# ChrisHird/ZLIB

Measured on AMD Instinct MI355X. Metric: GiB/s raw input compressed (deflate level 6), higher is better.
Workload: dtype u8

## Files before the change

zlib_amd/csrc/zgpu_lz_sorted.hip:

```cpp
#include "zgpu_common.h"
#include "zgpu_engine.h"
#define ZGPU_PARSE_HEADER_ONLY
#include "zgpu_lz_parse.h"
#include <cstdlib>
#include "../../include/zamd_gpu.h"

#include <atomic>
static std::atomic<int> g_inject_sort_fault{0};
extern "C" __attribute__((visibility("default"))) void zgpu_debug_inject_sort_fault(void) { g_inject_sort_fault.store(1); }

namespace zgpu {

__device__ inline uint32_t lds_off(const void *p) { return (uint32_t)(uintptr_t)(const __attribute__((address_space(3))) void *)p; }
__device__ inline void lds_st32(uint32_t a, uint32_t v) { asm volatile("ds_write_b32 %0, %1" ::"v"(a), "v"(v) : "memory"); }
__device__ inline void lds_st16(uint32_t a, uint32_t v) { asm volatile("ds_write_b16 %0, %1" ::"v"(a), "v"(v) : "memory"); }
__device__ inline void lds_max32(uint32_t a, uint32_t v) { asm volatile("ds_max_u32 %0, %1" ::"v"(a), "v"(v) : "memory"); }
__device__ inline uint32_t lds_ld32(uint32_t a) { uint32_t v; asm volatile("ds_read_b32 %0, %1\n\ts_waitcnt lgkmcnt(0)" : "=v"(v) : "v"(a) : "memory"); return v; }
__device__ inline uint32_t lds_ld16(uint32_t a) { uint32_t v; asm volatile("ds_read_u16 %0, %1\n\ts_waitcnt lgkmcnt(0)" : "=v"(v) : "v"(a) : "memory"); return v; }

__device__ inline void lds_st8(uint32_t a, uint32_t v) { asm volatile("ds_write_b8 %0, %1" ::"v"(a), "v"(v) : "memory"); }
__device__ inline uint32_t lds_ld8(uint32_t a) { uint32_t v; asm volatile("ds_read_u8 %0, %1\n\ts_waitcnt lgkmcnt(0)" : "=v"(v) : "v"(a) : "memory"); return v; }

constexpr uint32_t kSuperS = 1024;

// ... 514 lines not shown
    uint64_t lo; uint32_t n;
    chunk_span(g, c, lo, n);
    const uint8_t *src = g.in + lo;
    const uint16_t *S = S_all + (size_t)c * kSStride + kSPad;
    const unsigned long long *hd = reinterpret_cast<const unsigned long long *>(heads_all + (size_t)c * kHeadStride);
    uint2 *rec = recs + (size_t)c * kChunkMax;
    const uint32_t npos = n >= 3 ? n - 2 : 0;
    const uint32_t base = chunk_base(g, c);
    stage_chunk<kM2Threads>(src, n, d32, tid);
    if (tid == 0) *work_next = 0;
    for (uint32_t q2 = npos + tid; q2 < n; q2 += kM2Threads) rec[q2] = make_uint2((uint32_t)src[q2] << 24, 0);
    __syncthreads();

    const uint32_t chainF = cfg.chain, chainQ = cfg.chain >> 2, dbase = lds_off(d32), nblk = (npos + 63) >> 6;
    const uint16_t *hb = reinterpret_cast<const uint16_t *>(heads_all + (size_t)c * kHeadStride + kHeadWords);
    auto grab = [&]() { uint32_t b = 0; if (lane == 0) b = atomicAdd(work_next, 1u); return (uint32_t)__builtin_amdgcn_readfirstlane(b); };
    uint32_t blk = grab(), p_nx = 0, below_nx = 0;
    unsigned long long m_nx = 0;
    if (blk < nblk) { const uint32_t wi = (blk << 6) + lane; p_nx = wi < npos ? S[wi] : 0; m_nx = hd[blk]; below_nx = hb[blk]; }
    while (blk < nblk) {
        const uint32_t wi = (blk << 6) + lane;
        const bool valid = wi < npos;
        const uint32_t p = p_nx, below = below_nx;
        const unsigned long long m = m_nx;
        const uint32_t blk_nx = grab();
        if (blk_nx < nblk) { const uint32_t wn = (blk_nx << 6) + lane; p_nx = wn < npos ? S[wn] : 0; m_nx = hd[blk_nx]; below_nx = hb[blk_nx]; }
        uint32_t avail = 0;
        {
            const unsigned long long mine = m & ((2ull << lane) - 1);
            const uint32_t rank = mine ? (uint32_t)__builtin_clzll(mine) - (63 - lane) : lane + below;
            if (valid) avail = rank < chainF ? rank : chainF;
        }
        const int w = (int)(p + base);
        int thr = (w - (int)kMaxDist > 1 ? w - (int)kMaxDist : 1) - (int)base;
        const int thr_next = (w - (int)kMaxDist + 1 > 1 ? w - (int)kMaxDist + 1 : 1) - (int)base;
        if (cfg.strategy == kRle && thr < (int)p - 1) thr = (int)p - 1;
        uint32_t best = kMinMatch - 1, key_seen = 0, snapkey = 0;
        uint32_t scan2 = (uint32_t)d8[p + 1] | ((uint32_t)d8[p + 2] << 8);
        uint32_t boff = dbase + best - 1;
        unsigned long long amask = mask_gt_u32(avail, 0u);
        bool snap_taken = false;
        const uint16_t *sp = S + wi;
        lds_st32(slot + lane * 4, 0);
        lds_st16(pw + lane * 2, p);
        uint32_t tail = 0;
        const uint32_t lanebits = lane << 16, dummy = ring + (kRing - 1) * 4;
        M3_STAT(5, __popcll(__builtin_amdgcn_ballot_w64(valid)));

        auto fold = [&](uint32_t kcur) {
            const uint32_t cnt = tail < 64 ? tail : 64;
            M3_STAT(3, 1);
            tail = (uint32_t)__builtin_amdgcn_readfirstlane(tail - cnt);
            if (lane < cnt) {
                const uint32_t e = lds_ld32(ring + ((tail + lane) << 2));
                const uint32_t q = e & 0xffffu, o = (e >> 16) & 63u;
                const uint32_t k = kcur - ((kcur - (e >> 22)) & 1023u);
                const uint32_t po = lds_ld16(pw + o * 2), look = n - po, cap = look < kMaxMatch ? look : kMaxMatch, nice = cfg.nice < look ? cfg.nice : look;
                uint32_t l = 0, x;
                for (;;) {
                    x = lds_ld32u(dbase + q + l) ^ lds_ld32u(dbase + po + l);
                    M3_STAT(4, 1);
                    if (x != 0 || l + 4 >= cap) break;
                    l += 4;
                }
                uint32_t len = x ? l + ((uint32_t)__builtin_ctz(x) >> 3) : l + 4;
                len = len < cap ? len : cap;
                if (len >= kMinMatch) {
                    const uint32_t key = len >= nice ? (0x80000000u | ((4095u - k) << 16) | len) : ((len << 16) | (4095u - k));
                    lds_max32(slot + o * 4, key);
                }
            }
            const uint32_t key = lds_ld32(slot + lane * 4);
            if (key != key_seen) {
                key_seen = key;
                best = (key >> 31) ? key & 0x1ffu : key >> 16;
                boff = dbase + best - 1;
                scan2 = (uint32_t)d8[p + best - 1] | ((uint32_t)d8[p + best] << 8);
            }
            amask &= ~mask_lt_i32((int)key, 0);
        };

        auto group = [&](uint32_t k0) -> uint64_t {
            int gi = (int)wi - 4 - (int)k0, gsel;
            gi = gi < -(int)kSPad ? -(int)kSPad : gi;
            asm("v_cndmask_b32_e64 %0, %1, %2, %3" : "=v"(gsel) : "v"(-(int)kSPad), "v"(gi), "s"(amask));
            return reinterpret_cast<const U64u *>(S + gsel)->v;
        };
        uint64_t cq = group(0);
        uint32_t k = 0;
        const uint32_t snapK = chainQ & ~3u, snapJ = chainQ & 3u;
        for (;; k += 4) {
            if (amask == 0) break;
            if (k == chainQ) {
                while (tail) fold(k);
                snapkey = key_seen; snap_taken = true;
            } else if ((k & (ZGPU_M3_PERIOD - 1)) == 0) { while (tail) fold(k); }
            const uint64_t cqn = group(k + 4);
#pragma unroll
            for (uint32_t j = 0; j < 4; j++) {
                const uint32_t q = (uint32_t)(cq >> (48 - 16 * j)) & 0xffffu;
                if (j != 0 && j == snapJ && k == snapK) {
                    while (tail) fold(k + j);
                    snapkey = key_seen; snap_taken = true;
                }
                uint32_t b0, b1;
                lds_ld2bytes(boff + q, b0, b1);
                amask &= mask_le_i32(thr, (int)q);
                if (k == 0 && j == 0) thr = thr_next;
                const unsigned long long m = amask & mask_eq_u32(b0 | (b1 << 8), scan2);
                M3_STAT(0, 1); M3_STAT(1, __popcll(amask)); M3_STAT(2, __popcll(m));
                if (m) {
                    stack_push(m, (uint32_t)__builtin_amdgcn_readfirstlane(ring + (tail << 2)), dummy, q | lanebits | ((k + j) << 22));
                    tail = (uint32_t)__builtin_amdgcn_readfirstlane(tail + (uint32_t)__popcll(m));
                    if (tail >= 64) fold(k + j);
                }
                amask &= mask_gt_u32(avail, k + j + 1);
            }
            cq = cqn;
        }
        while (tail) fold(k);
        if (!snap_taken) snapkey = key_seen;
        if (valid) {
            uint32_t full = 0, snap = 0, flags = 0;
            if (key_seen) {
                const uint32_t kb = 4095u - ((key_seen >> 31) ? (key_seen >> 16) & 0xfffu : key_seen & 0xfffu);
                full = best | ((p - (uint32_t)sp[-1 - (int)kb]) << 9);
            }
            if (snapkey) {
                const uint32_t ks = 4095u - ((snapkey >> 31) ? (snapkey >> 16) & 0xfffu : snapkey & 0xfffu);
                const uint32_t sl = (snapkey >> 31) ? snapkey & 0x1ffu : snapkey >> 16;
                snap = sl | ((p - (uint32_t)sp[-1 - (int)ks]) << 9);
            }
            if (p + base == kWSize + kMaxDist && avail != 0 && (uint32_t)sp[-1] + base == kWSize) flags = 1;
            rec[p] = make_uint2(full | ((uint32_t)d8[p] << 24), snap | (flags << 24));
        }
        blk = blk_nx;
    }
}

#ifndef ZGPU_WTRIG
#define ZGPU_WTRIG 48
#endif
#ifndef ZGPU_WBLK
#define ZGPU_WBLK 64
#endif
#ifndef ZGPU_WNEU_SHIFT
#define ZGPU_WNEU_SHIFT 0
#endif
#ifndef ZGPU_WFOLD_AT
#define ZGPU_WFOLD_AT 64
#endif
constexpr uint32_t kWFoldAt = ZGPU_WFOLD_AT;
constexpr uint32_t kWThreads = 512, kWWaves = kWThreads / 64, kWBlk = ZGPU_WBLK, kWTrig = ZGPU_WTRIG, kWNeuShift = ZGPU_WNEU_SHIFT;
constexpr uint32_t kWNeuBytes = (kChunkMax >> kWNeuShift) / 8;
constexpr uint32_t kWOffLcnt = kM3DataLds + 16 + kWNeuBytes + kWWaves * kM3WaveLds;
constexpr uint32_t kWLds = kWOffLcnt + kP2Wins * 4;
static_assert(2 * kWLds <= 160 * 1024, "two walker workgroups per CU");
enum : uint32_t { W_NEED = 0, W_LIMBO = 1, W_READY = 2, W_SEARCH = 3, W_DONE = 4 };
#ifdef ZGPU_WALK_STATS
__device__ unsigned long long walk_stats[8];
extern "C" __attribute__((visibility("default"))) void zgpu_debug_walk_stats(unsigned long long *out, int reset)
{
    unsigned long long z[8] = {};
    hipMemcpyFromSymbol(out, HIP_SYMBOL(walk_stats), sizeof z);
    if (reset) hipMemcpyToSymbol(HIP_SYMBOL(walk_stats), z, sizeof z);
}
#define W_STAT(i, v) do { const unsigned long long v_ = (unsigned long long)(v); if (lane == 0) atomicAdd(&walk_stats[i], v_); } while (0)
__device__ unsigned long long walk_log_stats[2];
extern "C" __attribute__((visibility("default"))) void zgpu_debug_walk_log_stats(unsigned long long *out, int reset)
{
    unsigned long long z[2] = {};
    hipMemcpyFromSymbol(out, HIP_SYMBOL(walk_log_stats), sizeof z);
    if (reset) hipMemcpyToSymbol(HIP_SYMBOL(walk_log_stats), z, sizeof z);
}
#else
#define W_STAT(i, v) do { } while (0)
#endif
#ifdef ZGPU_WALK_TIME
__device__ unsigned long long walk_time[8];
extern "C" __attribute__((visibility("default"))) void zgpu_debug_walk_time(unsigned long long *out, int reset)
{
    unsigned long long z[8] = {};
    hipMemcpyFromSymbol(out, HIP_SYMBOL(walk_time), sizeof z);
    if (reset) hipMemcpyToSymbol(HIP_SYMBOL(walk_time), z, sizeof z);
}
#define W_T0() unsigned long long wt_prev = __builtin_readcyclecounter(), wt_fold = 0, wt_lds = 0, wt_take = 0, wt_acc[8] = {0, 0, 0, 0, 0, 0, 0, 0}
#define W_T(i) do { const unsigned long long t_ = __builtin_readcyclecounter(); wt_acc[i] += t_ - wt_prev - ((i) == 1 ? wt_fold + wt_lds + wt_take : 0); \
                    if ((i) == 1) { wt_acc[2] += wt_fold; wt_acc[3] += wt_lds; wt_acc[7] += wt_take; } wt_fold = wt_lds = wt_take = 0; wt_prev = t_; } while (0)
#define W_TF(stmt) do { const unsigned long long f0_ = __builtin_readcyclecounter(); stmt; wt_fold += __builtin_readcyclecounter() - f0_; } while (0)
#define W_TL(stmt) do { const unsigned long long f0_ = __builtin_readcyclecounter(); stmt; wt_lds += __builtin_readcyclecounter() - f0_; } while (0)
#define W_TK(stmt) do { const unsigned long long f0_ = __builtin_readcyclecounter(); asm volatile("s_waitcnt vmcnt(0)" ::: "memory"); stmt; wt_take += __builtin_readcyclecounter() - f0_; } while (0)
#define W_TEND() do { if (lane == 0) for (int i_ = 0; i_ < 8; i_++) atomicAdd(&walk_time[i_], wt_acc[i_]); } while (0)
#else
#define W_T0() do { } while (0)
#define W_T(i) do { } while (0)
#define W_TF(stmt) stmt
#define W_TL(stmt) stmt
#define W_TK(stmt) stmt
#define W_TEND() do { } while (0)
#endif
__device__ inline uint32_t add_w1(uint32_t b, uint32_t w) { uint32_t r; asm("v_add_u32_sdwa %0, %1, %2 dst_sel:DWORD dst_unused:UNUSED_PAD src0_sel:DWORD src1_sel:WORD_1" : "=v"(r) : "v"(b), "v"(w)); return r; }
__device__ inline uint32_t add_w0(uint32_t b, uint32_t w) { uint32_t r; asm("v_add_u32_sdwa %0, %1, %2 dst_sel:DWORD dst_unused:UNUSED_PAD src0_sel:DWORD src1_sel:WORD_0" : "=v"(r) : "v"(b), "v"(w)); return r; }
__device__ inline uint32_t or_w1(uint32_t b, uint32_t w) { uint32_t r; asm("v_or_b32_sdwa %0, %1, %2 dst_sel:DWORD dst_unused:UNUSED_PAD src0_sel:DWORD src1_sel:WORD_1" : "=v"(r) : "v"(b), "v"(w)); return r; }
__device__ inline uint32_t and_or(uint32_t w, uint32_t m, uint32_t b) { uint32_t r; asm("v_and_or_b32 %0, %1, %2, %3" : "=v"(r) : "v"(w), "s"(m), "v"(b)); return r; }
__device__ inline uint32_t sel_mask(unsigned long long m, uint32_t if_set, uint32_t if_clear) { uint32_t r; asm("v_cndmask_b32_e64 %0, %1, %2, %3" : "=v"(r) : "v"(if_clear), "v"(if_set), "s"(m)); return r; }

template <uint32_t T>
__device__ inline void tile_exits(uint8_t *pl, const uint32_t *gm, const uint32_t *gs, uint32_t h0, uint32_t h1, uint32_t nent, uint16_t *exits, uint32_t tid)
{
    constexpr uint32_t kWords = kChunkMax / 32;
    static_assert(kWords % T == 0 && T % 64 == 0 && T <= 1024, "workgroup size");
    uint32_t *HAS = reinterpret_cast<uint32_t *>(pl);
    uint16_t *wcnt = reinterpret_cast<uint16_t *>(pl + kWords * 4);
    uint32_t *wtot = reinterpret_cast<uint32_t *>(pl + kWords * 6);
    uint16_t *N = reinterpret_cast<uint16_t *>(pl + kWords * 6 + 64);
    constexpr uint32_t kCapNodes = (kM3DataLds - (kWords * 6 + 64)) / 2;
    static_assert(kCapNodes < 0x8000u && kCapNodes > kTileH1 / 3, "a path's game starts are three positions apart at least; different paths' need not be");
    const uint32_t lane = tid & 63, wave = tid >> 6;
    constexpr uint32_t per = kWords / T;
    uint32_t sum = 0, cnt[per];
#pragma unroll
    for (uint32_t i = 0; i < per; i++) {
        const uint32_t w = tid * per + i, v = __hip_atomic_load(gs + w, __ATOMIC_RELAXED, __HIP_MEMORY_SCOPE_AGENT);
        HAS[w] = v; cnt[i] = (uint32_t)__builtin_popcount(v); sum += cnt[i];
    }
    uint32_t x = sum;
#pragma unroll
    for (int d = 1; d < 64; d <<= 1) { const uint32_t y = __shfl_up(x, d); if ((int)lane >= d) x += y; }
    if (lane == 63) wtot[wave] = x;
    __syncthreads();
    uint32_t b = x - sum;
    for (uint32_t w = 0; w < wave; w++) b += wtot[w];
#pragma unroll
    for (uint32_t i = 0; i < per; i++) { wcnt[tid * per + i] = (uint16_t)b; b += cnt[i]; }
    __syncthreads();
    uint32_t nn = 0;
    for (uint32_t w = 0; w < T / 64; w++) nn += wtot[w];
    auto rank_of = [&](uint32_t p) { return (uint32_t)wcnt[p >> 5] + (uint32_t)__builtin_popcount(HAS[p >> 5] & ~(~0u << (p & 31u))); };
    if (nn > kCapNodes) {
        for (uint32_t k = tid; k < kTileExitStride; k += T) {
            uint32_t v = 0;
            if (k < nent) {
                const uint32_t e = h0 + k;
                uint32_t p = e < h1 ? next_bit(HAS, e, kWords) : kNone, x = e > h1 ? e : h1;
                while (p != kNone && p < h1) {
                    const uint32_t gv = __hip_atomic_load(gm + p, __ATOMIC_RELAXED, __HIP_MEMORY_SCOPE_AGENT), q = p + (gv >> 24) + ((gv >> 15) & 511u);
                    x = q > h1 ? q : h1;
                    p = q < h1 ? next_bit(HAS, q, kWords) : kNone;
                }
                v = x - h1;
            }
            exits[k] = (uint16_t)v;
        }
        return;
    }
    constexpr uint32_t kExit = 0x8000u;
    for (uint32_t p0 = h0 & ~31u; p0 < h1; p0 += T * 8) {
        uint32_t gv[8];
#pragma unroll
        for (uint32_t u = 0; u < 8; u++) { const uint32_t p = p0 + u * T + tid; gv[u] = p < h1 ? __hip_atomic_load(gm + p, __ATOMIC_RELAXED, __HIP_MEMORY_SCOPE_AGENT) : 0u; }
#pragma unroll
        for (uint32_t u = 0; u < 8; u++) {
            const uint32_t p = p0 + u * T + tid;
            if (p < h1 && ((HAS[p >> 5] >> (p & 31u)) & 1u)) {
                const uint32_t q = p + (gv[u] >> 24) + ((gv[u] >> 15) & 511u);
                uint32_t v = kExit | (q > h1 ? q - h1 : 0u);
                if (q < h1) { const uint32_t t = next_bit(HAS, q, kWords); if (t != kNone && t < h1) v = rank_of(t); }
                N[rank_of(p)] = (uint16_t)v;
            }
        }
    }
    __syncthreads();
    for (;;) {
        bool more = false;
        for (uint32_t i = tid; i < nn; i += T) {
            const uint32_t v = N[i];
            if (!(v & kExit)) { const uint32_t w = N[v]; N[i] = (uint16_t)w; more = more || !(w & kExit); }
        }
        if (!__syncthreads_or(more)) break;
    }
    for (uint32_t k = tid; k < kTileExitStride; k += T) {
        uint32_t v = 0;
        if (k < nent) {
            const uint32_t e = h0 + k, t = e < h1 ? next_bit(HAS, e, kWords) : kNone;
            v = (t == kNone || t >= h1) ? (e > h1 ? e - h1 : 0u) : ((uint32_t)N[rank_of(t)] & 0x7fffu);
        }
        exits[k] = (uint16_t)v;
    }
}

static_assert(kP2LogLdsBytes <= kWOffLcnt, "the parse works in the memory of the chunk bytes, the neutral bitmap and the rings");
template <int MODE>
__global__ void __launch_bounds__(kWThreads, kWThreads / 128) walk_kernel(ChunkGeom g, LevelCfg cfg, const uint16_t *__restrict__ S_all, const uint32_t *__restrict__ ir_all,
                                                            uint32_t *__restrict__ gm_all, uint32_t *__restrict__ gs_all, uint32_t *__restrict__ tokens, ChunkMeta *meta, TileGeom tg)
{
    static_assert(MODE == 1 || MODE == 2, "a chunk or a tile");
    constexpr bool FUSE = MODE == 1, TILE = MODE == 2;
    static_assert(!FUSE || kWNeuShift == 0, "a log holds kP2Win games: a position must start one game at most, so every neutral position is claimed");
    extern __shared__ __attribute__((aligned(16))) uint32_t lds[];
    uint32_t *d32 = lds;
    uint32_t *ctrl = lds + kM3DataLds / 4;
    uint32_t *NEU = ctrl + 4;
    uint32_t *lcnt = lds + kWOffLcnt / 4;
    const uint8_t *d8 = reinterpret_cast<const uint8_t *>(d32);
    const uint32_t c = blockIdx.x, tid = threadIdx.x, lane = tid & 63, wave = tid >> 6;
    const uint32_t ring = (uint32_t)__builtin_amdgcn_readfirstlane(lds_off(lds) + kM3DataLds + 16 + kWNeuBytes + wave * kM3WaveLds), slot = ring + kRing * 4, pw = slot + 64 * 4;
    uint64_t lo; uint32_t n;
    chunk_span(g, c, lo, n);
    const uint8_t *src = g.in + lo;
    const uint16_t *S = S_all + (size_t)c * kSStride + kSPad;
    const uint32_t *ir = ir_all + (size_t)c * kChunkMax;
    uint32_t *gm = gm_all + (size_t)c * kChunkMax, *gs = gs_all + (size_t)c * (kChunkMax / 32);
    uint32_t *lrec = gm; uint16_t *lpos = reinterpret_cast<uint16_t *>(gs_all) + (size_t)c * kChunkMax;
    uint32_t th0 = 0, th1 = n, tnent = 0, tnent_all = 0, nil_local = ~0u;
    uint32_t base = chunk_base(g, c);
    if (TILE) {
        uint64_t wb; uint32_t nl;
        tile_span(g, tg, c, wb, nl, th0, th1, tnent);
        tnent_all = tnent;
        if (tnent > th1 - th0) tnent = th1 - th0;
        base = (tg.abs0_nil && tg.abs0 + wb == 0) ? 0u : 1u;
        if (tg.nil_pos >= wb && tg.nil_pos - wb < kChunkMax) nil_local = (uint32_t)(tg.nil_pos - wb);
    }
    const uint32_t npos = n >= 3 ? n - 2 : 0;
    stage_chunk<kWThreads>(src, n, d32, tid);
    for (uint32_t i = tid; i < kChunkMax / 32; i += kWThreads) { if (i < kWNeuBytes / 4) NEU[i] = 0; if (!FUSE) gs[i] = 0; }
    if (tid < 8) d32[(kChunkMax + 64) / 4 + tid] = 0xffffffffu;
    if (tid == 0) ctrl[0] = 0;
    if (FUSE && tid < kP2Wins) lcnt[tid] = 0;
    __syncthreads();
    int slide_at;
    {
        const int room = (int)(2 * kWSize - base), b0 = (int)n < room ? (int)n : room;
        const int a = b0 - (int)kMinLookahead + 1, b = (int)(kWSize + kMaxDist) - (int)base;
        slide_at = a > b ? a : b;
    }
    const uint32_t chainF = cfg.chain, chainQ = cfg.chain >> 2, dbase = lds_off(d32), nblk = TILE ? tnent + (th1 - th0 - tnent + kWBlk - 1) / kWBlk : (n + kWBlk - 1) / kWBlk;
    const uint32_t wlim = TILE ? th1 : n;
    const bool vexact = (chainF & 7u) != 0 || (chainQ & 7u) != 0 || cfg.strategy == kRle;
    uint32_t lanebits = lane << 16;
    const uint32_t dummy = ring + (kRing - 1) * 4;
    uint32_t st = W_NEED, x = 0, handL = kMinMatch - 1, handM = 0, handD = 0, gstart = 0;
    uint32_t irx = 0, irn = 0, irE = 0, irl = 0;
    bool haveE = false;
    uint32_t rem = 0, best = kMinMatch - 1, key_seen = 0, sentinel = 0, scan2 = 0, boff = dbase + 1;
    int gi = -(int)kSPad;
    uint32_t firstb = 0;
    uint4 G0 = make_uint4(0, 0, 0, 0), G1 = G0, G2 = G0, G3 = G0, F0 = G0, F1 = G0, F2 = G0, F3 = G0;
    uint32_t left = 0;
    bool cont = false;
    unsigned long long amask = 0, jmask = 0;
    uint32_t tail = 0;

    auto fold = [&]() {
        const uint32_t cnt = tail < 64 ? tail : 64;
        W_STAT(5, 1); W_STAT(6, cnt);
        tail = (uint32_t)__builtin_amdgcn_readfirstlane(tail - cnt);
        if (lane < cnt) {
            const uint32_t e = lds_ld32(ring + ((tail + lane) << 2));
            const uint32_t q = e & 0xffffu, o = (e >> 16) & 63u;
            const uint32_t po = lds_ld16(pw + o * 2), look = n - po, cap = look < kMaxMatch ? look : kMaxMatch, nice = cfg.nice < look ? cfg.nice : look;
            const bool reach = po - q <= kMaxDist - ((e >> 22) & 1u ? 0u : 1u) && q + base >= 1u;
            uint32_t l = 0, xa, xb;
            for (;;) {
                lds_cmp8(dbase + q + l, dbase + po + l, xa, xb);
                if ((xa | xb) != 0 || l + 8 >= cap) break;
                l += 8;
            }
            uint32_t len = xa ? l + ((uint32_t)__builtin_ctz(xa) >> 3) : xb ? l + 4 + ((uint32_t)__builtin_ctz(xb) >> 3) : l + 8;
            len = len < cap ? len : cap;
            if (len >= kMinMatch && reach) lds_max32(slot + o * 4, (len >= nice && len > (e >> 23)) ? (0x80000000u | (q << 9) | len) : ((len << 16) | q));
        }
        const uint32_t key = lds_ld32(slot + lane * 4);
        if (key != key_seen) {
            key_seen = key;
            best = (key >> 31) ? key & 0x1ffu : key >> 16;
            boff = dbase + best - 1;
            scan2 = (uint32_t)d8[x + best - 1] | ((uint32_t)d8[x + best] << 16);
        }
        amask &= ~mask_lt_i32((int)key, 0);
    };
    auto gload = [&](int gi) -> uint4 { gi = gi < -(int)kSPad ? -(int)kSPad : gi; return reinterpret_cast<const U128u *>(S + gi)->v; };

    W_T0();
    W_T(3);
    for (;;) {
        while (tail) fold();
        W_T(4);
        if (cont && (key_seen >> 31)) cont = false;
        const bool fin = st == W_SEARCH && !(((amask | jmask) >> lane) & 1ull) && !cont;
        W_STAT(2, 1); W_STAT(3, __popcll(__builtin_amdgcn_ballot_w64(fin || st == W_LIMBO || st == W_NEED)));
        if (st == W_LIMBO) { irx = irl; st = W_READY; }
        uint32_t y = 0, irY = 0;
        bool toN = false, haveIr = false;
        if (fin) {
            uint32_t len = kMinMatch - 1, dist = 0;
            if (key_seen != sentinel) {
                const bool nz = key_seen >> 31;
                len = nz ? key_seen & 0x1ffu : key_seen >> 16;
                dist = x - (nz ? (key_seen >> 9) & 0xffffu : key_seen & 0xffffu);
            }
            if (len <= 5 && (cfg.strategy == kFiltered || (len == kMinMatch && dist > kTooFar))) len = kMinMatch - 1;
            bool emit = false;
            if (len > handL) {
                if (handL < kMinMatch) gstart = x;
                handL = len; handD = dist; handM = x;
                if (len < cfg.lazy && x + 1 < npos) { x = x + 1; irx = irn; st = W_READY; }
                else emit = true;
                haveE = false;
            } else if (handL >= kMinMatch) emit = true;
            else { y = x + 1; irY = irn; toN = haveIr = true; }
            if (emit) {
                const uint32_t rec = ((handM - gstart) << 24) | (handL << 15) | handD;
                if (FUSE) {
                    const uint32_t w = gstart / kP2Win, at = w * kP2Win + atomicAdd(&lcnt[w], 1u);
                    lrec[at] = rec; lpos[at] = (uint16_t)gstart;
                } else {
                    gm[gstart] = rec;
                    atomicOr(&gs[gstart >> 5], 1u << (gstart & 31u));
                }
                y = handM + handL; irY = irE; haveIr = haveE; toN = true;
                handL = kMinMatch - 1;
            }
        }
        if (toN) {
            st = W_NEED;
            if (y < wlim) {
                const uint32_t yc = y >> kWNeuShift, bit = 1u << (yc & 31u);
                const bool meet = (y & ((1u << kWNeuShift) - 1u)) == 0;
                if (!meet || !(atomicOr(&NEU[yc >> 5], bit) & bit)) {
                    x = y;
                    if (haveIr) { irx = irY; st = W_READY; }
                    else { irl = y < npos ? ir[y] : 0; st = W_LIMBO; W_STAT(7, 1); }
                }
            }
        }
        W_T(5);
        {
            const unsigned long long nm = __builtin_amdgcn_ballot_w64(st == W_NEED);
            if (nm) {
                const int first = __builtin_ctzll(nm);
                uint32_t b0 = 0;
                if ((int)lane == first) b0 = atomicAdd(&ctrl[0], (uint32_t)__popcll(nm));
                b0 = (uint32_t)__builtin_amdgcn_readlane((int)b0, first);
                if (st == W_NEED) {
                    const uint32_t b = b0 + __builtin_amdgcn_mbcnt_hi((uint32_t)(nm >> 32), __builtin_amdgcn_mbcnt_lo((uint32_t)nm, 0));
                    if (b >= nblk) st = W_DONE;
                    else {
                        const uint32_t y2 = TILE ? (b < tnent ? th0 + b : th0 + tnent + (b - tnent) * kWBlk) : b * kWBlk, bit = 1u << ((y2 >> kWNeuShift) & 31u);
                        if (!(atomicOr(&NEU[(y2 >> kWNeuShift) >> 5], bit) & bit)) { x = y2; handL = kMinMatch - 1; irl = y2 < npos ? ir[y2] : 0; st = W_LIMBO; }
                    }
                }
            }
        }
        W_T(6);
        bool fresh = false;
        if (st == W_READY) {
            const uint32_t seed = handL, idx = irx & 0xffffu, rank = irx >> 16, budget = seed >= cfg.good ? (chainQ ? chainQ : 0xffffu) : chainF;
            uint32_t avail = (x < npos && seed < cfg.lazy) ? (rank < budget ? rank : budget) : 0;
            irn = x + 1 < npos ? ir[x + 1] : 0;
            if (seed >= kMinMatch) { const uint32_t E = handM + handL; irE = E < npos ? ir[E] : 0; haveE = true; }
            if (TILE) {
                if (x == nil_local && avail != 0 && x - (uint32_t)S[idx - 1] == kMaxDist) avail = 0;
                if (cfg.strategy == kHuffmanOnly) avail = 0;
                if (cfg.strategy == kRle && avail != 0) avail = x - (uint32_t)S[idx - 1] == 1 ? 1u : 0u;
            }
            else if (x + base == kWSize + kMaxDist && avail != 0 && (int)x >= slide_at && (uint32_t)S[idx - 1] + base == kWSize) avail = 0;
            best = seed; sentinel = (seed << 16) | 0xffffu; key_seen = sentinel; boff = dbase + best - 1;
            scan2 = (uint32_t)d8[x + best - 1] | ((uint32_t)d8[x + best] << 16);
            lds_st32(slot + lane * 4, sentinel);
            lds_st16(pw + lane * 2, x);
            lanebits = (lane << 16) | (seed << 23);
            rem = avail; firstb = 1u << 22;
            gi = (int)idx - 8;
            st = W_SEARCH;
            fresh = avail != 0;
            W_STAT(4, 1);
        }
        if (cont) { cont = false; fresh = true; }
        jmask = __builtin_amdgcn_ballot_w64(fresh);
        if (fresh) {
            F0 = gload(gi);
            if (rem > 8) F1 = gload(gi - 8);
            if (rem > 16) F2 = gload(gi - 16);
            if (rem > 24) F3 = gload(gi - 24);
            gi -= 32;
        }
        W_T(0);
        if (__builtin_amdgcn_ballot_w64(st != W_DONE) == 0) { W_TEND(); break; }
        const unsigned long long smask = __builtin_amdgcn_ballot_w64(st == W_SEARCH);
        const uint32_t idle = (uint32_t)__popcll(__builtin_amdgcn_ballot_w64(st == W_LIMBO || st == W_NEED));

        for (bool first = true;; first = false) {
            const unsigned long long amask0 = amask;
            if (amask) {
                W_STAT(0, 1);
                const uint32_t scan0 = sel_mask(amask0, scan2, 0xffffffffu);
                uint32_t bb[8], a[8], boff_e;
                boff_e = boff;
                if (!vexact) {
                    const uint32_t boff_i = dbase + kChunkMax + 8u;
                    G0.x = sel_mask(amask0, G0.x, 0u); G0.y = sel_mask(amask0, G0.y, 0u); G0.z = sel_mask(amask0, G0.z, 0u); G0.w = sel_mask(amask0, G0.w, 0u);
                    boff_e = sel_mask(amask0, boff, boff_i);
                }
                a[0] = add_w1(boff_e, G0.w); a[1] = add_w0(boff_e, G0.w); a[2] = add_w1(boff_e, G0.z); a[3] = add_w0(boff_e, G0.z);
                a[4] = add_w1(boff_e, G0.y); a[5] = add_w0(boff_e, G0.y); a[6] = add_w1(boff_e, G0.x); a[7] = add_w0(boff_e, G0.x);
                if (vexact) {
                    const uint32_t nv = rem < 8 ? rem : 8, sent = dbase + (scan2 ? kChunkMax + 8u : kChunkMax + 64u + 8u);
#pragma unroll
                    for (uint32_t j = 0; j < 8; j++) a[j] = j < nv ? a[j] : sent;
                }
                uint32_t hi[8];
                W_TL(
                    asm volatile("ds_read_u8 %0, %16\n\tds_read_u8 %8, %16 offset:1\n\tds_read_u8 %1, %17\n\tds_read_u8 %9, %17 offset:1\n\t"
                                 "ds_read_u8 %2, %18\n\tds_read_u8 %10, %18 offset:1\n\tds_read_u8 %3, %19\n\tds_read_u8 %11, %19 offset:1\n\t"
                                 "ds_read_u8 %4, %20\n\tds_read_u8 %12, %20 offset:1\n\tds_read_u8 %5, %21\n\tds_read_u8 %13, %21 offset:1\n\t"
                                 "ds_read_u8 %6, %22\n\tds_read_u8 %14, %22 offset:1\n\tds_read_u8 %7, %23\n\tds_read_u8 %15, %23 offset:1\n\t"
                                 "s_waitcnt lgkmcnt(0)"
                                 : "=&v"(bb[0]), "=&v"(bb[1]), "=&v"(bb[2]), "=&v"(bb[3]), "=&v"(bb[4]), "=&v"(bb[5]), "=&v"(bb[6]), "=&v"(bb[7]),
                                   "=&v"(hi[0]), "=&v"(hi[1]), "=&v"(hi[2]), "=&v"(hi[3]), "=&v"(hi[4]), "=&v"(hi[5]), "=&v"(hi[6]), "=&v"(hi[7])
                                 : "v"(a[0]), "v"(a[1]), "v"(a[2]), "v"(a[3]), "v"(a[4]), "v"(a[5]), "v"(a[6]), "v"(a[7]) : "memory"));
#pragma unroll
                for (uint32_t j = 0; j < 8; j++) bb[j] |= hi[j] << 16;
                W_STAT(1, __popcll(amask0) * 8);
                const uint32_t lf = lanebits | firstb;
                unsigned long long mm[8];
                uint32_t total = 0;
#pragma unroll
                for (uint32_t j = 0; j < 8; j++) { mm[j] = mask_eq_u32(bb[j], scan0); total += (uint32_t)__popcll(mm[j]); }
                auto entry_of = [&](uint32_t j) -> uint32_t {
                    const uint32_t wd = j < 2 ? G0.w : j < 4 ? G0.z : j < 6 ? G0.y : G0.x, lb = j == 0 ? lf : lanebits;
                    return (j & 1) ? and_or(wd, 0xffffu, lb) : or_w1(lb, wd);
                };
                if (total) {
                    if (tail + total > kRing - 1) { while (tail) W_TF(fold()); }
                    if (total <= kRing - 1) {
                        uint32_t ta[8], te[8];
#pragma unroll
                        for (uint32_t j = 0; j < 8; j++) {
                            ta[j] = stack_slot(mm[j], ring + (tail << 2)); te[j] = entry_of(j);
                            tail += (uint32_t)__popcll(mm[j]);
                        }
                        tail = (uint32_t)__builtin_amdgcn_readfirstlane(tail);
                        unsigned long long sv;
                        asm volatile("s_mov_b64 %0, exec\n\t"
                                     "s_mov_b64 exec, %17\n\tds_write_b32 %1, %9\n\ts_mov_b64 exec, %18\n\tds_write_b32 %2, %10\n\t"
                                     "s_mov_b64 exec, %19\n\tds_write_b32 %3, %11\n\ts_mov_b64 exec, %20\n\tds_write_b32 %4, %12\n\t"
                                     "s_mov_b64 exec, %21\n\tds_write_b32 %5, %13\n\ts_mov_b64 exec, %22\n\tds_write_b32 %6, %14\n\t"
                                     "s_mov_b64 exec, %23\n\tds_write_b32 %7, %15\n\ts_mov_b64 exec, %24\n\tds_write_b32 %8, %16\n\t"
                                     "s_mov_b64 exec, %0"
                                     : "=&s"(sv)
                                     : "v"(ta[0]), "v"(ta[1]), "v"(ta[2]), "v"(ta[3]), "v"(ta[4]), "v"(ta[5]), "v"(ta[6]), "v"(ta[7]),
                                       "v"(te[0]), "v"(te[1]), "v"(te[2]), "v"(te[3]), "v"(te[4]), "v"(te[5]), "v"(te[6]), "v"(te[7]),
                                       "s"(mm[0]), "s"(mm[1]), "s"(mm[2]), "s"(mm[3]), "s"(mm[4]), "s"(mm[5]), "s"(mm[6]), "s"(mm[7]) : "memory");
                    } else {
#pragma unroll
                        for (uint32_t j = 0; j < 8; j++) {
                            if (mm[j]) {
                                stack_push(mm[j], (uint32_t)__builtin_amdgcn_readfirstlane(ring + (tail << 2)), dummy, entry_of(j));
                                tail = (uint32_t)__builtin_amdgcn_readfirstlane(tail + (uint32_t)__popcll(mm[j]));
                                if (tail >= kWFoldAt) W_TF(fold());
                            }
                        }
                    }
                    while (tail >= kWFoldAt) W_TF(fold());
                }
                amask &= mask_gt_u32(rem, 8u);
                firstb = sel_mask(amask0, 0u, firstb);
            }
            G0 = G1; G1 = G2; G2 = G3;
            left = left ? left - 1 : 0;
            if (first && jmask) {
                W_TK(if ((jmask >> lane) & 1ull) { G0 = F0; G1 = F1; G2 = F2; G3 = F3; left = 4; });
            }
            rem = sel_mask(amask0, rem > 8 ? rem - 8 : 0, rem);
            {
                const unsigned long long cm = amask & mask_eq_u32(left, 0u);
                cont = cont || ((cm >> lane) & 1ull);
                amask &= ~cm;
            }
            amask |= jmask; jmask = 0;
            if (amask == 0 || (uint32_t)__popcll(smask & ~amask) + idle >= kWTrig) break;
        }
        W_T(1);
    }
    if (TILE) {
        __syncthreads();
        tile_exits<kWThreads>(reinterpret_cast<uint8_t *>(lds), gm, gs, th0, th1, tnent_all, tg.exits + (size_t)c * kTileExitStride, tid);
    }
    if (FUSE) {
        __syncthreads();
#ifdef ZGPU_WALK_STATS
        if (tid < kP2Wins) { atomicAdd(&walk_log_stats[0], (unsigned long long)lcnt[tid]); atomicMax(&walk_log_stats[1], (unsigned long long)lcnt[tid]); }
#endif
        constexpr uint32_t kP2Threads = kWThreads;
        constexpr bool LITE = true, FUSED = true, TILE = false, LOG = true;
        const uint2 *recs = nullptr;
        const uint32_t *gmv_all = nullptr, *gsv_all = nullptr;
        uint8_t *pl = reinterpret_cast<uint8_t *>(lds);
        uint16_t *const J = reinterpret_cast<uint16_t *>(pl + kP2OffJ);
        uint32_t *const HAS = reinterpret_cast<uint32_t *>(pl + kP2OffHAS), *const MARK = reinterpret_cast<uint32_t *>(pl + kP2OffMARK), *const COV = reinterpret_cast<uint32_t *>(pl + kP2OffCOV),
                 *const MAT = reinterpret_cast<uint32_t *>(pl + kP2OffMAT), *const wbase = reinterpret_cast<uint32_t *>(pl + kP2OffWbase), *const VIS = reinterpret_cast<uint32_t *>(pl + kP2OffVIS),
                 *const EXITS = reinterpret_cast<uint32_t *>(pl + kP2OffEXITS), *const wave_tot = reinterpret_cast<uint32_t *>(pl + kP2OffWtot);
        uint32_t &sh_entry = *reinterpret_cast<uint32_t *>(pl + kP2OffEntry), &sh_exit = *reinterpret_cast<uint32_t *>(pl + kP2OffEntry + 4);
        uint16_t *const END = reinterpret_cast<uint16_t *>(pl + kP2OffEND);
#include "zgpu_lz_parse_body.inc"
    }
}

struct __attribute__((packed, aligned(1))) U128b { uint4 v; };
enum : uint32_t { F_IR = 0, F_GROUP, F_CAND, F_EXT, F_DONE };

__device__ inline uint32_t first_diff16(uint4 a, uint4 b)
{
    const uint64_t x0 = (((uint64_t)(a.y ^ b.y)) << 32) | (a.x ^ b.x), x1 = (((uint64_t)(a.w ^ b.w)) << 32) | (a.z ^ b.z);
    return x0 ? (uint32_t)__builtin_ctzll(x0) >> 3 : x1 ? 8 + ((uint32_t)__builtin_ctzll(x1) >> 3) : 16u;
}

__device__ __noinline__ uint4 tail16(const uint8_t *in, uint32_t o, uint64_t safe_end)
{
    uint32_t v[4] = {0, 0, 0, 0};
    for (uint32_t k = 0; k < 16 && (uint64_t)o + k < safe_end; k++) v[k >> 2] |= (uint32_t)in[o + k] << (8 * (k & 3));
    return make_uint4(v[0], v[1], v[2], v[3]);
}

__global__ void __launch_bounds__(64) fast_kernel(ChunkGeom g, LevelCfg cfg, const uint16_t *__restrict__ S_all, const uint32_t *__restrict__ ir_all, uint8_t *G_all,
                                                   uint32_t *__restrict__ tokens, ChunkMeta *meta, uint32_t lanes)
{
    const uint32_t c = blockIdx.x * lanes + threadIdx.x;
    const bool live = threadIdx.x < lanes && c < g.nchunks;
    const uint32_t cc = live ? c : 0;
    uint64_t lo; uint32_t n;
    chunk_span(g, cc, lo, n);
    const uint8_t *in = g.in + lo;
    const uint64_t safe_end = g.in_bytes - lo;
    const uint16_t *S = S_all + (size_t)cc * kSStride + kSPad;
    const uint32_t *ir = ir_all + (size_t)cc * kChunkMax;
    uint8_t *G = G_all + (size_t)cc * kGStride + kGPad;
    uint32_t *tok = tokens + (size_t)cc * kChunkMax;
    const uint8_t *dummy = reinterpret_cast<const uint8_t *>(S_all);
    const uint32_t base = chunk_base(g, cc);
    uint32_t off = 0, ntok = 0, blk_tok0 = 0, nblk = 0, nostore = 0, block_start = 0;
    auto cut_block = [&](uint32_t p_end) {
        if (off != 0 && block_start + base < kWSize) nostore |= 1u << nblk;
        nblk++; blk_tok0 = ntok; block_start = p_end;
    };
    const uint32_t room = 2 * kWSize - base;
    uint32_t buffered = n < room ? n : room;
    uint32_t p = 0, st = live ? F_IR : F_DONE;
    auto token_top = [&]() {
        if (buffered - p < kMinLookahead) {
            if ((int)(p + base) - (int)off >= (int)(kWSize + kMaxDist)) off += kWSize;
            buffered = n;
            if (n == p) { cut_block(p); st = F_DONE; }
        }
    };
    if (live) token_top();
    uint32_t irw[8] = {0, 0, 0, 0, 0, 0, 0, 0};
    uint4 scan = make_uint4(0, 0, 0, 0), cb[4] = {scan, scan, scan, scan};
    bool fresh = false;
    uint32_t idx = 0, rank = 0, j0 = 0, chain = 0, best = 0, mstart = 0, cap = 0, nice = 0, look = 0, ncand = 0, cand[4] = {0, 0, 0, 0}, extl = 0;
    int w = 0, limit = 0;
    bool first = true, over = false, lastg = false;

    auto setup_search = [&](uint32_t iv) {
        idx = iv & 0xffffu; rank = iv >> 16;
        w = (int)(p + base) - (int)off; limit = w > (int)kMaxDist ? w - (int)kMaxDist : 0;
        cap = look < kMaxMatch ? look : kMaxMatch; nice = cfg.nice < look ? cfg.nice : look;
        chain = cfg.chain; best = kMinMatch - 1; first = true; over = false; lastg = false; j0 = 0; ncand = 0;
    };

    for (;;) {
        if (__builtin_amdgcn_ballot_w64(st != F_DONE) == 0) break;
        constexpr uint32_t kNone = 0xffffffffu;
        const uint8_t *a0 = dummy, *a1 = dummy, *a2 = dummy, *a3 = dummy;
        uint32_t o0 = kNone, o1 = kNone, o2 = kNone, o3 = kNone, o4 = kNone;
        const bool want_ir = st == F_IR || (st == F_GROUP && fresh);
        if (want_ir) { a2 = reinterpret_cast<const uint8_t *>(ir + p); a3 = reinterpret_cast<const uint8_t *>(ir + p + 4); o4 = p; }
        if (st == F_GROUP) { const int at = (int)idx - (int)j0 - 8; a0 = reinterpret_cast<const uint8_t *>(S + at); a1 = G + at; }
        if (st == F_CAND) { o0 = cand[0]; o1 = ncand > 1 ? cand[1] : kNone; o2 = ncand > 2 ? cand[2] : kNone; o3 = ncand > 3 ? cand[3] : kNone; }
        if (st == F_EXT) { o0 = cand[0] + extl; o1 = p + extl; }
        const bool u0 = o0 != kNone && (uint64_t)o0 + 16 > safe_end, u1 = o1 != kNone && (uint64_t)o1 + 16 > safe_end, u2 = o2 != kNone && (uint64_t)o2 + 16 > safe_end,
                   u3 = o3 != kNone && (uint64_t)o3 + 16 > safe_end, u4 = o4 != kNone && (uint64_t)o4 + 16 > safe_end;
        if (o0 != kNone && !u0) a0 = in + o0;
        if (o1 != kNone && !u1) a1 = in + o1;
        if (o2 != kNone && !u2) a2 = in + o2;
        if (o3 != kNone && !u3) a3 = in + o3;
        const uint8_t *a4 = (o4 != kNone && !u4) ? in + o4 : dummy;
        uint4 r0 = reinterpret_cast<const U128b *>(a0)->v, r1 = reinterpret_cast<const U128b *>(a1)->v, r2 = reinterpret_cast<const U128b *>(a2)->v,
              r3 = reinterpret_cast<const U128b *>(a3)->v, r4 = reinterpret_cast<const U128b *>(a4)->v;
        if (__builtin_amdgcn_ballot_w64(u0 || u1 || u2 || u3 || u4)) {
            if (u0) r0 = tail16(in, o0, safe_end);
            if (u1) r1 = tail16(in, o1, safe_end);
            if (u2) r2 = tail16(in, o2, safe_end);
            if (u3) r3 = tail16(in, o3, safe_end);
            if (u4) r4 = tail16(in, o4, safe_end);
        }

        bool eval = false, fin = false;
        if (want_ir) {
            irw[0] = r2.x; irw[1] = r2.y; irw[2] = r2.z; irw[3] = r2.w; irw[4] = r3.x; irw[5] = r3.y; irw[6] = r3.z; irw[7] = r3.w;
            scan = r4;
        }
        if (st == F_IR) {
            look = n - p;
            if (look < kMinMatch) { first = true; fin = true; }
            else { setup_search(irw[0]); if (rank == 0) fin = true; else st = F_GROUP; }
        } else if (st == F_GROUP) {
            fresh = false;
            const uint64_t fl = ((uint64_t)r1.y << 32) | r1.x;
            uint32_t used = 0;
            const uint32_t room4 = chain < 4 ? chain : 4;
            for (uint32_t t = 0; t < 8; t++) {
                if (ncand >= room4) break;
                if (j0 + t + 1 > rank) { lastg = true; break; }
                used = t + 1;
                const uint32_t slot = 7 - t;
                if (!((fl >> (8 * slot)) & 1u)) continue;
                const uint32_t wd = slot >= 6 ? r0.w : slot >= 4 ? r0.z : slot >= 2 ? r0.y : r0.x, q = (slot & 1) ? wd >> 16 : wd & 0xffffu;
                const int wq = (int)(q + base) - (int)off;
                bool stop = wq <= 0;
                if (first) { stop = stop || (uint32_t)(w - wq) > kMaxDist; first = first && stop; }
                else stop = stop || wq <= limit;
                if (stop) { lastg = true; break; }
                cand[3] = ncand == 3 ? q : cand[3]; cand[2] = ncand == 2 ? q : cand[2]; cand[1] = ncand == 1 ? q : cand[1]; cand[0] = ncand == 0 ? q : cand[0];
                ncand++;
            }
            j0 += used;
            if (ncand) st = F_CAND;
            else if (lastg || j0 >= rank) fin = true;
        } else if (st == F_CAND) {
            cb[0] = r0; cb[1] = r1; cb[2] = r2; cb[3] = r3;
            eval = true;
        } else if (st == F_EXT) {
            const uint32_t d = first_diff16(r0, r1);
            extl += d;
            if (d < 16 || extl >= cap) { st = F_CAND; eval = true; }
        }
        if (eval) {
            uint32_t l = st == F_CAND && extl ? extl : 0;
            bool known = extl != 0;
            extl = 0;
            while (ncand != 0) {
                if (!known) { l = first_diff16(cb[0], scan); if (l == 16 && cap > 16) { st = F_EXT; extl = 16; break; } }
                known = false;
                l = l < cap ? l : cap;
                bool end = false;
                if (l > best) { mstart = cand[0]; best = l; end = l >= nice; }
                end = end || --chain == 0;
                cand[0] = cand[1]; cand[1] = cand[2]; cand[2] = cand[3]; cb[0] = cb[1]; cb[1] = cb[2]; cb[2] = cb[3]; ncand--;
                if (end) { fin = true; ncand = 0; }
            }
            if (st == F_CAND && !fin) { if (lastg || j0 >= rank) fin = true; else st = F_GROUP; }
        }
        if (fin) {
            uint32_t L = 1;
            const uint32_t match_len = first ? kMinMatch - 1 : (best <= look ? best : look);
            if (look >= kMinMatch) G[idx] = 1;
            if (match_len >= kMinMatch) {
                tok[ntok++] = tok_match(p - mstart, match_len - kMinMatch);
                if (match_len <= cfg.lazy && look - match_len >= kMinMatch) {
#pragma unroll
                    for (uint32_t k = 1; k < 7; k++) if (k < match_len) G[irw[k] & 0xffffu] = 1;
                }
                L = match_len;
            } else tok[ntok++] = tok_lit(scan.x & 255u);
            const bool cut = ntok - blk_tok0 == kBlockTokens;
            p += L;
            if (cut) cut_block(p);
            st = F_IR; extl = 0; ncand = 0;
            token_top();
            if (st != F_DONE && L < 8 && n - p >= kMinMatch) {
                uint32_t iv = irw[1];
#pragma unroll
                for (uint32_t k = 2; k < 8; k++) iv = L == k ? irw[k] : iv;
                if ((iv >> 16) != 0) { look = n - p; setup_search(iv); fresh = true; st = F_GROUP; }
            }
        }
    }
    if (live) { meta[c].ntok = ntok; meta[c].nostore = nostore; meta[c].in_bytes = n; }
}

static bool launch_sort(const ChunkGeom &g, const SortedWs &ws, ChunkMeta *meta, hipStream_t st, zgpu_engine *prof, int exact_sort)
{
    static int sort_env = -1;
    if (sort_env < 0) { const char *e = getenv("ZGPU_SORT"); sort_env = e ? atoi(e) : 4; }
    const bool exact = exact_sort || sort_env == 1;
    hipEvent_t ev{};
    prof_span_begin(prof, st, &ev);
    if (exact) {
        hipLaunchKernelGGL(sort_kernel, dim3(g.nchunks), dim3(kSortThreads), 0, st, g, ws.S, ws.rk, ws.heads, ws.ir);
        hipLaunchKernelGGL(heads_below_kernel, dim3(g.nchunks), dim3(1024), 0, st, ws.heads);
    } else {
        hipLaunchKernelGGL(sort4_kernel, dim3(g.nchunks), dim3(kS4Threads), 0, st, g, ws.S, ws.heads, ws.fault, ws.ir, meta);
        if (g_inject_sort_fault.exchange(0)) hipMemsetAsync(ws.fault, 1, 4, st);
    }
    prof_span_end(prof, st, ZGPU_STAGE_CHAIN, ev);
    return !exact;
}

template <int MODE> static void launch_walk(const ChunkGeom &g, LevelCfg cfg, const SortedWs &ws, uint32_t *tokens, ChunkMeta *meta, const TileGeom &tg, hipStream_t st)
{
    static bool opt_in = false;
    if (!opt_in) { hipFuncSetAttribute(reinterpret_cast<const void *>(walk_kernel<MODE>), hipFuncAttributeMaxDynamicSharedMemorySize, (int)kWLds); opt_in = true; }
    uint32_t *games = MODE == 1 ? ws.lrec() : ws.gm(), *starts = MODE == 1 ? reinterpret_cast<uint32_t *>(ws.lpos()) : ws.gs();
    hipLaunchKernelGGL(walk_kernel<MODE>, dim3(g.nchunks), dim3(kWThreads), kWLds, st, g, cfg, ws.S, ws.ir, games, starts, tokens, meta, tg);
}

bool launch_lz_sorted(const ChunkGeom &g, LevelCfg cfg, void *workspace, uint32_t *tokens, ChunkMeta *meta, hipStream_t st, zgpu_engine *prof, int exact_sort, int impl)
{
    const SortedWs ws(workspace, g.nchunks);
    const bool adler_done = launch_sort(g, ws, meta, st, prof, exact_sort);
    hipEvent_t ev{};
    prof_span_begin(prof, st, &ev);
    if (impl == ZGPU_LZ_FASTWIN) launch_lz_fastwin(g, cfg, ws.S, ws.ir, tokens, meta, st);
    else if (impl == ZGPU_LZ_FAST) {
        hipMemsetAsync(ws.G(), 0, ws.nch * kGStride, st);
        static int forced = -1;
        if (forced < 0) { const char *v = getenv("ZGPU_FAST_LANES"); forced = v ? atoi(v) : 0; if (forced < 0 || forced > 64) forced = 0; }
        uint32_t lanes = (uint32_t)forced;
        if (!lanes) { lanes = 1; while (lanes < 64 && (uint64_t)lanes * 4096 < g.nchunks) lanes <<= 1; }
        hipLaunchKernelGGL(fast_kernel, dim3((g.nchunks + lanes - 1) / lanes), dim3(64), 0, st, g, cfg, ws.S, ws.ir, ws.G(), tokens, meta, lanes);
    } else if (impl == ZGPU_LZ_WALK) launch_walk<1>(g, cfg, ws, tokens, meta, TileGeom{}, st);
    else {
        static bool opt_in3 = false;
        if (!opt_in3) { hipFuncSetAttribute(reinterpret_cast<const void *>(match3_kernel), hipFuncAttributeMaxDynamicSharedMemorySize, (int)kM3Lds); opt_in3 = true; }
        hipLaunchKernelGGL(match3_kernel, dim3(g.nchunks), dim3(kM2Threads), kM3Lds, st, g, cfg, ws.S, ws.heads, ws.recs);
        prof_span_end(prof, st, ZGPU_STAGE_MATCH, ev);
        prof_span_begin(prof, st, &ev);
        launch_parse(g, cfg, ws.recs, tokens, meta, st);
        prof_span_end(prof, st, ZGPU_STAGE_PARSE, ev);
        return adler_done;
// ... 36 lines not shown
```

Baseline: 28.90.

## Batch LDS ops in walk kernel and share lane state via bpermute

```diff
diff --git a/zlib_amd/csrc/zgpu_lz_sorted.hip b/zlib_amd/csrc/zgpu_lz_sorted.hip
--- a/zlib_amd/csrc/zgpu_lz_sorted.hip
+++ b/zlib_amd/csrc/zgpu_lz_sorted.hip
@@ -840,9 +840,8 @@
     uint32_t *ctrl = lds + kM3DataLds / 4;
     uint32_t *NEU = ctrl + 4;
     uint32_t *lcnt = lds + kWOffLcnt / 4;
-    const uint8_t *d8 = reinterpret_cast<const uint8_t *>(d32);
     const uint32_t c = blockIdx.x, tid = threadIdx.x, lane = tid & 63, wave = tid >> 6;
-    const uint32_t ring = (uint32_t)__builtin_amdgcn_readfirstlane(lds_off(lds) + kM3DataLds + 16 + kWNeuBytes + wave * kM3WaveLds), slot = ring + kRing * 4, pw = slot + 64 * 4;
+    const uint32_t ring = (uint32_t)__builtin_amdgcn_readfirstlane(lds_off(lds) + kM3DataLds + 16 + kWNeuBytes + wave * kM3WaveLds), slot = ring + kRing * 4;
     uint64_t lo; uint32_t n;
     chunk_span(g, c, lo, n);
     const uint8_t *src = g.in + lo;
@@ -881,7 +880,8 @@
     uint32_t st = W_NEED, x = 0, handL = kMinMatch - 1, handM = 0, handD = 0, gstart = 0;
     uint32_t irx = 0, irn = 0, irE = 0, irl = 0;
     bool haveE = false;
-    uint32_t rem = 0, best = kMinMatch - 1, key_seen = 0, sentinel = 0, scan2 = 0, boff = dbase + 1;
+    uint32_t rem = 0, best = kMinMatch - 1, key_seen = 0, sentinel = 0, boff = dbase + 1;
+    uint32_t sw0 = 0, sw1 = 0;
     int gi = -(int)kSPad;
     uint32_t firstb = 0;
     uint4 G0 = make_uint4(0, 0, 0, 0), G1 = G0, G2 = G0, G3 = G0, F0 = G0, F1 = G0, F2 = G0, F3 = G0;
@@ -894,16 +894,24 @@
         const uint32_t cnt = tail < 64 ? tail : 64;
         W_STAT(5, 1); W_STAT(6, cnt);
         tail = (uint32_t)__builtin_amdgcn_readfirstlane(tail - cnt);
+        const uint32_t e = lds_ld32(ring + ((tail + lane) << 2));
+        const uint32_t q = e & 0xffffu, o = (e >> 16) & 63u, qa = dbase + q;
+        uint32_t po, xa, xb;
+        {
+            uint64_t va; uint32_t va2, ow0, ow1;
+            asm volatile("ds_bpermute_b32 %0, %5, %6\n\tds_bpermute_b32 %1, %5, %7\n\tds_bpermute_b32 %2, %5, %8\n\t"
+                         "ds_read2_b32 %3, %9 offset1:1\n\tds_read_b32 %4, %9 offset:8\n\ts_waitcnt lgkmcnt(0)"
+                         : "=&v"(po), "=&v"(ow0), "=&v"(ow1), "=&v"(va), "=&v"(va2) : "v"(o << 2), "v"(x), "v"(sw0), "v"(sw1), "v"(qa & ~3u) : "memory");
+            xa = __builtin_amdgcn_alignbyte((uint32_t)(va >> 32), (uint32_t)va, qa & 3) ^ ow0;
+            xb = __builtin_amdgcn_alignbyte(va2, (uint32_t)(va >> 32), qa & 3) ^ ow1;
+        }
         if (lane < cnt) {
-            const uint32_t e = lds_ld32(ring + ((tail + lane) << 2));
-            const uint32_t q = e & 0xffffu, o = (e >> 16) & 63u;
-            const uint32_t po = lds_ld16(pw + o * 2), look = n - po, cap = look < kMaxMatch ? look : kMaxMatch, nice = cfg.nice < look ? cfg.nice : look;
+            const uint32_t look = n - po, cap = look < kMaxMatch ? look : kMaxMatch, nice = cfg.nice < look ? cfg.nice : look;
             const bool reach = po - q <= kMaxDist - ((e >> 22) & 1u ? 0u : 1u) && q + base >= 1u;
-            uint32_t l = 0, xa, xb;
-            for (;;) {
-                lds_cmp8(dbase + q + l, dbase + po + l, xa, xb);
-                if ((xa | xb) != 0 || l + 8 >= cap) break;
+            uint32_t l = 0;
+            while ((xa | xb) == 0 && l + 8 < cap) {
                 l += 8;
+                lds_cmp8(qa + l, dbase + po + l, xa, xb);
             }
             uint32_t len = xa ? l + ((uint32_t)__builtin_ctz(xa) >> 3) : xb ? l + 4 + ((uint32_t)__builtin_ctz(xb) >> 3) : l + 8;
             len = len < cap ? len : cap;
@@ -914,7 +922,6 @@
             key_seen = key;
             best = (key >> 31) ? key & 0x1ffu : key >> 16;
             boff = dbase + best - 1;
-            scan2 = (uint32_t)d8[x + best - 1] | ((uint32_t)d8[x + best] << 16);
         }
         amask &= ~mask_lt_i32((int)key, 0);
     };
@@ -929,8 +936,8 @@
         const bool fin = st == W_SEARCH && !(((amask | jmask) >> lane) & 1ull) && !cont;
         W_STAT(2, 1); W_STAT(3, __popcll(__builtin_amdgcn_ballot_w64(fin || st == W_LIMBO || st == W_NEED)));
         if (st == W_LIMBO) { irx = irl; st = W_READY; }
-        uint32_t y = 0, irY = 0;
-        bool toN = false, haveIr = false;
+        uint32_t y = 0, irY = 0, rec = 0;
+        bool toN = false, haveIr = false, emit = false;
         if (fin) {
             uint32_t len = kMinMatch - 1, dist = 0;
             if (key_seen != sentinel) {
@@ -939,7 +946,6 @@
                 dist = x - (nz ? (key_seen >> 9) & 0xffffu : key_seen & 0xffffu);
             }
             if (len <= 5 && (cfg.strategy == kFiltered || (len == kMinMatch && dist > kTooFar))) len = kMinMatch - 1;
-            bool emit = false;
             if (len > handL) {
                 if (handL < kMinMatch) gstart = x;
                 handL = len; handD = dist; handM = x;
@@ -949,11 +955,8 @@
             } else if (handL >= kMinMatch) emit = true;
             else { y = x + 1; irY = irn; toN = haveIr = true; }
             if (emit) {
-                const uint32_t rec = ((handM - gstart) << 24) | (handL << 15) | handD;
-                if (FUSE) {
-                    const uint32_t w = gstart / kP2Win, at = w * kP2Win + atomicAdd(&lcnt[w], 1u);
-                    lrec[at] = rec; lpos[at] = (uint16_t)gstart;
-                } else {
+                rec = ((handM - gstart) << 24) | (handL << 15) | handD;
+                if (!FUSE) {
                     gm[gstart] = rec;
                     atomicOr(&gs[gstart >> 5], 1u << (gstart & 31u));
                 }
@@ -961,16 +964,31 @@
                 handL = kMinMatch - 1;
             }
         }
+        const uint32_t yc = y >> kWNeuShift, ybit = 1u << (yc & 31u);
+        const bool meet = (y & ((1u << kWNeuShift) - 1u)) == 0;
+        const bool claim = toN && y < wlim && meet;
+        const uint32_t own = ring + lane * 4, lw = gstart / kP2Win;
+        const uint32_t xs = dbase + (toN ? y : x);
+        uint32_t lslot = 0, yold, tw2; uint64_t tw;
+        if (FUSE) {
+            asm volatile("ds_add_rtn_u32 %0, %4, %5\n\tds_or_rtn_b32 %1, %6, %7\n\tds_read2_b32 %2, %8 offset1:1\n\tds_read_b32 %3, %8 offset:8\n\ts_waitcnt lgkmcnt(0)"
+                         : "=&v"(lslot), "=&v"(yold), "=&v"(tw), "=&v"(tw2)
+                         : "v"(emit ? lds_off(lcnt) + lw * 4 : own), "v"(emit ? 1u : 0u), "v"(claim ? lds_off(NEU) + (yc >> 5) * 4 : own), "v"(claim ? ybit : 0u), "v"(xs & ~3u) : "memory");
+        } else {
+            asm volatile("ds_or_rtn_b32 %0, %3, %4\n\tds_read2_b32 %1, %5 offset1:1\n\tds_read_b32 %2, %5 offset:8\n\ts_waitcnt lgkmcnt(0)"
+                         : "=&v"(yold), "=&v"(tw), "=&v"(tw2) : "v"(claim ? lds_off(NEU) + (yc >> 5) * 4 : own), "v"(claim ? ybit : 0u), "v"(xs & ~3u) : "memory");
+        }
+        const uint32_t tw0 = __builtin_amdgcn_alignbyte((uint32_t)(tw >> 32), (uint32_t)tw, xs & 3), tw1 = __builtin_amdgcn_alignbyte(tw2, (uint32_t)(tw >> 32), xs & 3);
+        if (FUSE && emit) {
+            const uint32_t at = lw * kP2Win + lslot;
+            lrec[at] = rec; lpos[at] = (uint16_t)gstart;
+        }
         if (toN) {
             st = W_NEED;
-            if (y < wlim) {
-                const uint32_t yc = y >> kWNeuShift, bit = 1u << (yc & 31u);
-                const bool meet = (y & ((1u << kWNeuShift) - 1u)) == 0;
-                if (!meet || !(atomicOr(&NEU[yc >> 5], bit) & bit)) {
-                    x = y;
-                    if (haveIr) { irx = irY; st = W_READY; }
-                    else { irl = y < npos ? ir[y] : 0; st = W_LIMBO; W_STAT(7, 1); }
-                }
+            if (y < wlim && (!meet || !(yold & ybit))) {
+                x = y;
+                if (haveIr) { irx = irY; st = W_READY; }
+                else { irl = y < npos ? ir[y] : 0; st = W_LIMBO; W_STAT(7, 1); }
             }
         }
         W_T(5);
@@ -1005,9 +1023,8 @@
             }
             else if (x + base == kWSize + kMaxDist && avail != 0 && (int)x >= slide_at && (uint32_t)S[idx - 1] + base == kWSize) avail = 0;
             best = seed; sentinel = (seed << 16) | 0xffffu; key_seen = sentinel; boff = dbase + best - 1;
-            scan2 = (uint32_t)d8[x + best - 1] | ((uint32_t)d8[x + best] << 16);
             lds_st32(slot + lane * 4, sentinel);
-            lds_st16(pw + lane * 2, x);
+            sw0 = tw0; sw1 = tw1;
             lanebits = (lane << 16) | (seed << 23);
             rem = avail; firstb = 1u << 22;
             gi = (int)idx - 8;
@@ -1033,39 +1050,41 @@
             const unsigned long long amask0 = amask;
             if (amask) {
                 W_STAT(0, 1);
-                const uint32_t scan0 = sel_mask(amask0, scan2, 0xffffffffu);
-                uint32_t bb[8], a[8], boff_e;
-                boff_e = boff;
+                uint32_t bb[8], a[8], boff_e, as;
+                boff_e = boff; as = boff + x;
                 if (!vexact) {
                     const uint32_t boff_i = dbase + kChunkMax + 8u;
                     G0.x = sel_mask(amask0, G0.x, 0u); G0.y = sel_mask(amask0, G0.y, 0u); G0.z = sel_mask(amask0, G0.z, 0u); G0.w = sel_mask(amask0, G0.w, 0u);
-                    boff_e = sel_mask(amask0, boff, boff_i);
+                    boff_e = sel_mask(amask0, boff, boff_i); as = sel_mask(amask0, as, boff_i + 64u);
                 }
                 a[0] = add_w1(boff_e, G0.w); a[1] = add_w0(boff_e, G0.w); a[2] = add_w1(boff_e, G0.z); a[3] = add_w0(boff_e, G0.z);
                 a[4] = add_w1(boff_e, G0.y); a[5] = add_w0(boff_e, G0.y); a[6] = add_w1(boff_e, G0.x); a[7] = add_w0(boff_e, G0.x);
-                if (vexact) {
-                    const uint32_t nv = rem < 8 ? rem : 8, sent = dbase + (scan2 ? kChunkMax + 8u : kChunkMax + 64u + 8u);
-#pragma unroll
-                    for (uint32_t j = 0; j < 8; j++) a[j] = j < nv ? a[j] : sent;
-                }
-                uint32_t hi[8];
+                uint32_t hi[8], s0, s1;
                 W_TL(
-                    asm volatile("ds_read_u8 %0, %16\n\tds_read_u8 %8, %16 offset:1\n\tds_read_u8 %1, %17\n\tds_read_u8 %9, %17 offset:1\n\t"
-                                 "ds_read_u8 %2, %18\n\tds_read_u8 %10, %18 offset:1\n\tds_read_u8 %3, %19\n\tds_read_u8 %11, %19 offset:1\n\t"
-                                 "ds_read_u8 %4, %20\n\tds_read_u8 %12, %20 offset:1\n\tds_read_u8 %5, %21\n\tds_read_u8 %13, %21 offset:1\n\t"
-                                 "ds_read_u8 %6, %22\n\tds_read_u8 %14, %22 offset:1\n\tds_read_u8 %7, %23\n\tds_read_u8 %15, %23 offset:1\n\t"
+                    asm volatile("ds_read_u8 %0, %18\n\tds_read_u8 %8, %18 offset:1\n\tds_read_u8 %1, %19\n\tds_read_u8 %9, %19 offset:1\n\t"
+                                 "ds_read_u8 %2, %20\n\tds_read_u8 %10, %20 offset:1\n\tds_read_u8 %3, %21\n\tds_read_u8 %11, %21 offset:1\n\t"
+                                 "ds_read_u8 %4, %22\n\tds_read_u8 %12, %22 offset:1\n\tds_read_u8 %5, %23\n\tds_read_u8 %13, %23 offset:1\n\t"
+                                 "ds_read_u8 %6, %24\n\tds_read_u8 %14, %24 offset:1\n\tds_read_u8 %7, %25\n\tds_read_u8 %15, %25 offset:1\n\t"
+                                 "ds_read_u8 %16, %26\n\tds_read_u8 %17, %26 offset:1\n\t"
                                  "s_waitcnt lgkmcnt(0)"
                                  : "=&v"(bb[0]), "=&v"(bb[1]), "=&v"(bb[2]), "=&v"(bb[3]), "=&v"(bb[4]), "=&v"(bb[5]), "=&v"(bb[6]), "=&v"(bb[7]),
-                                   "=&v"(hi[0]), "=&v"(hi[1]), "=&v"(hi[2]), "=&v"(hi[3]), "=&v"(hi[4]), "=&v"(hi[5]), "=&v"(hi[6]), "=&v"(hi[7])
-                                 : "v"(a[0]), "v"(a[1]), "v"(a[2]), "v"(a[3]), "v"(a[4]), "v"(a[5]), "v"(a[6]), "v"(a[7]) : "memory"));
+                                   "=&v"(hi[0]), "=&v"(hi[1]), "=&v"(hi[2]), "=&v"(hi[3]), "=&v"(hi[4]), "=&v"(hi[5]), "=&v"(hi[6]), "=&v"(hi[7]), "=&v"(s0), "=&v"(s1)
+                                 : "v"(a[0]), "v"(a[1]), "v"(a[2]), "v"(a[3]), "v"(a[4]), "v"(a[5]), "v"(a[6]), "v"(a[7]), "v"(as) : "memory"));
 #pragma unroll
                 for (uint32_t j = 0; j < 8; j++) bb[j] |= hi[j] << 16;
+                const uint32_t scan0 = s0 | (s1 << 16);
                 W_STAT(1, __popcll(amask0) * 8);
                 const uint32_t lf = lanebits | firstb;
                 unsigned long long mm[8];
                 uint32_t total = 0;
 #pragma unroll
-                for (uint32_t j = 0; j < 8; j++) { mm[j] = mask_eq_u32(bb[j], scan0); total += (uint32_t)__popcll(mm[j]); }
+                for (uint32_t j = 0; j < 8; j++) mm[j] = mask_eq_u32(bb[j], scan0);
+                if (vexact) {
+#pragma unroll
+                    for (uint32_t j = 0; j < 8; j++) mm[j] &= amask0 & mask_gt_u32(rem, j);
+                }
+#pragma unroll
+                for (uint32_t j = 0; j < 8; j++) total += (uint32_t)__popcll(mm[j]);
                 auto entry_of = [&](uint32_t j) -> uint32_t {
                     const uint32_t wd = j < 2 ? G0.w : j < 4 ? G0.z : j < 6 ? G0.y : G0.x, lb = j == 0 ? lf : lanebits;
                     return (j & 1) ? and_or(wd, 0xffffu, lb) : or_w1(lb, wd);
```

Measured after the change: 29.39 (median of 6 runs). 1.7% higher.
